# mryab/learning-at-home

Hardware: NVIDIA H100
Metric: DMoE training samples/sec (whole job, device-timed, max over ranks) (higher is better)
Workload: dtype bf16

## Files before the change

### learning-at-home_b200/csrc/small_m.cu

```cuda
#include "sm90.cuh"
#include <climits>

namespace lah {
namespace smallm {

constexpr int BM = 128;
constexpr int BK = 64;
constexpr int MMA_K = 16;
constexpr int BN_MAX = 128;
constexpr int NUM_THREADS = 288;

namespace sab {

constexpr int STAGES = 6;
constexpr int A_BYTES = BM * BK * 2;
constexpr int B_BYTES = BN_MAX * BK * 2;
constexpr int STAGE_BYTES = A_BYTES + B_BYTES;
constexpr int BAR_OFFSET = STAGES * STAGE_BYTES;
constexpr int QD = 4;
constexpr int MAX_G = 1023;
constexpr int CUM_OFFSET = BAR_OFFSET + (2 * STAGES + 2 * QD) * 8 + QD * 4 + 16;
constexpr int SMEM_TOTAL = CUM_OFFSET + (MAX_G + 1) * 4 + 1024;
static_assert(SMEM_TOTAL <= 232448, "shared memory budget");

struct Params {
    int G, M_out, K;
    const int* group_off;
    const int* group_rows;
    bf16* out;
    long long ldo;
    const float* bias;
    const bf16* residual;
    long long ldr;
    const int* wait_flags;
    int wait_count, wait_epoch;
    const int* epoch_base;
    int* status;
    int* tile_counter;
};

__device__ __forceinline__ int box_rows_of(int nn) { return nn <= 16 ? 16 : (nn <= 32 ? 32 : (nn <= 64 ? 64 : 128)); }

__device__ __forceinline__ int find_group(const int* cum, int G, int gc) {
    int lo = 0, hi = G - 1;
    while (lo < hi) {
        const int mid = (lo + hi + 1) >> 1;
        if (cum[mid] <= gc) lo = mid; else hi = mid - 1;
    }
    return lo;
}

template <int NB, bool A_MN>
__device__ __forceinline__ void sab_tile(const Params& p, uint8_t* smem, uint64_t* full_bar, uint64_t* empty_bar, int& stage,
                                         uint32_t& phase, int num_kb, int wg, int warp, int lane, int g, int ms, int row0,
// ... 141 lines not shown
                mbar_wait(&empty_bar[stage], phase ^ 1);
                uint8_t* sa = smem + stage * STAGE_BYTES;
                uint8_t* sb = sa + A_BYTES;
                const int k = kb * BK;
                mbar_arrive_expect_tx(&full_bar[stage], A_BYTES + box * 128);
                if (!A_MN) {
                    tma_load_3d(sa, &tmA, &full_bar[stage], k, ms * BM, g);
                } else {
#pragma unroll
                    for (int i = 0; i < BM / 64; ++i)
                        tma_load_3d(sa + i * (BK * 128), &tmA, &full_bar[stage], ms * BM + i * 64, k, g);
                }
                tma_load_2d(sb, tmB, &full_bar[stage], k, off + n0);
                if (++stage == STAGES) {
                    stage = 0;
                    phase ^= 1;
                }
            }
        }
        return;
    }

    const int wg = warp >> 2;
    int stage = 0, qi = 0;
    uint32_t phase = 0, qphase = 0;
    while (true) {
        mbar_wait(&q_full[qi], qphase);
        const int tile = q_tile[qi];
        __syncwarp();
        if (lane == 0) mbar_arrive(&q_empty[qi]);
        if (++qi == QD) {
            qi = 0;
            qphase ^= 1;
        }
        if (tile >= total) break;
        const int gc = tile / m_slices, ms = tile - gc * m_slices;
        const int g = find_group(cum, p.G, gc);
        const int n0 = (gc - cum[g]) * BN_MAX;
        const int nn = min(__ldg(p.group_rows + g) - n0, BN_MAX);
        const int row0 = __ldg(p.group_off + g) + n0;
        switch (box_rows_of(nn)) {
            case 16: sab_tile<16, A_MN>(p, smem, full_bar, empty_bar, stage, phase, num_kb, wg, warp, lane, g, ms, row0, nn); break;
            case 32: sab_tile<32, A_MN>(p, smem, full_bar, empty_bar, stage, phase, num_kb, wg, warp, lane, g, ms, row0, nn); break;
            case 64: sab_tile<64, A_MN>(p, smem, full_bar, empty_bar, stage, phase, num_kb, wg, warp, lane, g, ms, row0, nn); break;
            default: sab_tile<128, A_MN>(p, smem, full_bar, empty_bar, stage, phase, num_kb, wg, warp, lane, g, ms, row0, nn); break;
        }
    }
}

}

namespace wa {

constexpr int WBK = 32;
constexpr int OP_STAGES = 2;
constexpr int OP_STAGE_BYTES = 2 * (WBK * BM * 2);
constexpr int OP_BYTES = OP_STAGES * OP_STAGE_BYTES;
constexpr int CH_COLS = 32;
constexpr int CHUNKS = BN_MAX / CH_COLS;
constexpr int ARR_BYTES = BM * CH_COLS * 4;
constexpr int ST_STAGES = 3;
constexpr int ST_STAGE_BYTES = 4 * ARR_BYTES;
constexpr int ST_OFFSET = OP_BYTES;
constexpr int BAR_OFFSET = ST_OFFSET + ST_STAGES * ST_STAGE_BYTES;
constexpr int QD = 4;
constexpr int SMEM_TOTAL = BAR_OFFSET + (2 * OP_STAGES + 2 * ST_STAGES + 2 * QD) * 8 + QD * 4 + 16 + 1024;
static_assert(ST_STAGES <= CHUNKS, "the producer issues a tile's first ST_STAGES chunks before its remaining k-blocks");
static_assert(OP_STAGE_BYTES % 1024 == 0 && ARR_BYTES % 1024 == 0, "128-B swizzle atoms need 1 KB alignment");
static_assert(SMEM_TOTAL <= 232448, "shared memory budget");

struct Params {
    int G, N, K;
    const int* group_off;
    const int* group_rows;
    const int* skip;
    const int* step;
    float* p;
    float* m;
    float* v;
    float* vmax;
    bf16* p_bf16;
    float lr, beta1, beta2, eps;
    int amsgrad;
    float wd;
    int* tile_counter;
    const int* poison;
};

constexpr int WD_NONE = 0, WD_L2 = 1, WD_DECOUPLED = 2;

struct Tile {
    int g, mt, nt;
};

struct StateMaps {
    CUtensorMap a[4];
};

template <int WD>
__global__ void __launch_bounds__(NUM_THREADS, 1)
wgrad_adam_kernel(const Params p, const __grid_constant__ CUtensorMap tmDY, const __grid_constant__ CUtensorMap tmX,
                  const __grid_constant__ StateMaps tmS) {
    extern __shared__ uint8_t smem_raw[];
    uint8_t* smem = reinterpret_cast<uint8_t*>((reinterpret_cast<uintptr_t>(smem_raw) + 1023) & ~uintptr_t(1023));
    uint8_t* st_smem = smem + ST_OFFSET;
    uint64_t* op_full = reinterpret_cast<uint64_t*>(smem + BAR_OFFSET);
    uint64_t* op_empty = op_full + OP_STAGES;
    uint64_t* st_full = op_empty + OP_STAGES;
    uint64_t* st_empty = st_full + ST_STAGES;
    uint64_t* q_full = st_empty + ST_STAGES;
    uint64_t* q_empty = q_full + QD;
    volatile int* q_tile = reinterpret_cast<volatile int*>(q_empty + QD);

    const int warp = threadIdx.x >> 5;
    const int lane = threadIdx.x & 31;
    if (p.poison && (*p.poison & 1)) return;
    const int n_arr = p.amsgrad ? 4 : 3;

    if (warp == 8 && lane == 0) {
        tma_prefetch_desc(&tmDY);
        tma_prefetch_desc(&tmX);
        for (int a = 0; a < n_arr; ++a) tma_prefetch_desc(&tmS.a[a]);
        for (int i = 0; i < OP_STAGES; ++i) {
            mbar_init(&op_full[i], 1);
            mbar_init(&op_empty[i], 8);
        }
        for (int i = 0; i < ST_STAGES; ++i) {
            mbar_init(&st_full[i], 1);
            mbar_init(&st_empty[i], 1);
        }
        for (int i = 0; i < QD; ++i) {
            mbar_init(&q_full[i], 1);
            mbar_init(&q_empty[i], 8);
        }
        fence_mbar_init();
    }
    __syncthreads();

    const int n_tiles = p.K / BN_MAX;
    const int tiles_per_group = (p.N / BM) * n_tiles;
    const int total = p.G * tiles_per_group;
    auto decode = [&](int tile) {
        Tile t;
        t.g = tile / tiles_per_group;
        const int r = tile - t.g * tiles_per_group;
        t.mt = r / n_tiles;
        t.nt = r - t.mt * n_tiles;
        return t;
    };

    if (warp == 8) {
        if (lane != 0) return;
        uint32_t phase = 0, qphase = 0, sphase = 0;
        int qi = 0, stage = 0, sstage = 0;
        while (true) {
            int tile;
            while (true) {
                tile = atomicAdd(p.tile_counter, 1);
                if (tile >= total) break;
                const int g = tile / tiles_per_group;
                if (__ldg(p.group_rows + g) > 0 && !(p.skip && __ldg(p.skip + 2 * g) >= 0)) break;
                atomicMax(p.tile_counter, (g + 1) * tiles_per_group);
            }
            mbar_wait(&q_empty[qi], qphase ^ 1);
            q_tile[qi] = tile;
            mbar_arrive(&q_full[qi]);
            if (++qi == QD) {
                qi = 0;
                qphase ^= 1;
            }
            if (tile >= total) break;
            const Tile t = decode(tile);
            const int off = __ldg(p.group_off + t.g), rows = __ldg(p.group_rows + t.g);
            const int srow = t.g * p.N + t.mt * BM;
            auto load_chunk = [&](int c) {
                mbar_wait(&st_empty[sstage], sphase ^ 1);
                mbar_arrive_expect_tx(&st_full[sstage], n_arr * ARR_BYTES);
                uint8_t* ss = st_smem + sstage * ST_STAGE_BYTES;
                for (int a = 0; a < n_arr; ++a)
                    tma_load_2d(ss + a * ARR_BYTES, &tmS.a[a], &st_full[sstage], t.nt * BN_MAX + c * CH_COLS, srow);
                if (++sstage == ST_STAGES) {
                    sstage = 0;
                    sphase ^= 1;
                }
            };
            for (int t0 = 0; t0 < rows; t0 += WBK) {
                mbar_wait(&op_empty[stage], phase ^ 1);
                mbar_arrive_expect_tx(&op_full[stage], OP_STAGE_BYTES);
                uint8_t* sa = smem + stage * OP_STAGE_BYTES;
                uint8_t* sb = sa + WBK * BM * 2;
#pragma unroll
                for (int i = 0; i < BM / 64; ++i)
                    tma_load_2d(sa + i * (WBK * 128), &tmDY, &op_full[stage], t.mt * BM + i * 64, off + t0);
#pragma unroll
                for (int i = 0; i < BN_MAX / 64; ++i)
                    tma_load_2d(sb + i * (WBK * 128), &tmX, &op_full[stage], t.nt * BN_MAX + i * 64, off + t0);
                if (++stage == OP_STAGES) {
                    stage = 0;
                    phase ^= 1;
                }
                if (t0 == 0)
                    for (int c = 0; c < ST_STAGES; ++c) load_chunk(c);
            }
            for (int c = ST_STAGES; c < CHUNKS; ++c) load_chunk(c);
        }
        return;
    }

    const int wg = warp >> 2;
    int qi = 0, stage = 0, sstage = 0;
    uint32_t phase = 0, qphase = 0, sphase = 0;
    float acc[BN_MAX / 2];
    const int lrow = wg * 64 + (warp & 3) * 16 + (lane >> 2);
    const int sw = lrow & 7;
    while (true) {
        mbar_wait(&q_full[qi], qphase);
        const int tile = q_tile[qi];
        __syncwarp();
        if (lane == 0) mbar_arrive(&q_empty[qi]);
        if (++qi == QD) {
            qi = 0;
            qphase ^= 1;
        }
        if (tile >= total) break;
        const Tile t = decode(tile);
        const int rows = __ldg(p.group_rows + t.g);
        int prev_stage = -1;
        for (int t0 = 0; t0 < rows; t0 += WBK) {
            mbar_wait(&op_full[stage], phase);
            const uint32_t sa = smem_u32(smem + stage * OP_STAGE_BYTES) + wg * (WBK * 128);
            const uint32_t sb = smem_u32(smem + stage * OP_STAGE_BYTES + WBK * BM * 2);
            const int ksteps = min(WBK / MMA_K, (rows - t0 + MMA_K - 1) / MMA_K);
            wgmma_fence();
            for (int k = 0; k < ksteps; ++k) {
                const uint64_t da = make_smem_desc_sw128(sa + k * (MMA_K * 128), WBK * 128, 1024);
                const uint64_t db = make_smem_desc_sw128(sb + k * (MMA_K * 128), WBK * 128, 1024);
                wgmma_bf16_n128<1, 1>(acc, da, db, (t0 > 0 || k > 0) ? 1u : 0u);
            }
            wgmma_commit();
            wgmma_wait<1>();
            if (prev_stage >= 0) {
                __syncwarp();
                if (lane == 0) mbar_arrive(&op_empty[prev_stage]);
            }
            prev_stage = stage;
            if (++stage == OP_STAGES) {
                stage = 0;
                phase ^= 1;
            }
        }
        wgmma_wait<0>();
        wgmma_fence_regs(acc);
        __syncwarp();
        if (lane == 0 && prev_stage >= 0) mbar_arrive(&op_empty[prev_stage]);

        const float st = static_cast<float>(__ldg(p.step + t.g));
        const float step_size = p.lr / (1.f - powf(p.beta1, st));
        const float inv_sqrt_bc2 = rsqrtf(1.f - powf(p.beta2, st));
        const int srow = t.g * p.N + t.mt * BM;
        const long long row_base = static_cast<long long>(srow) + lrow;
        const int col_base = t.nt * BN_MAX + 2 * (lane & 3);
#pragma unroll
        for (int c = 0; c < CHUNKS; ++c) {
            mbar_wait(&st_full[sstage], sphase);
            uint8_t* ss = st_smem + sstage * ST_STAGE_BYTES;
#pragma unroll
            for (int jj = 0; jj < CH_COLS / 8; ++jj)
#pragma unroll
                for (int h = 0; h < 2; ++h) {
                    const int so = (lrow + 8 * h) * 128 + (((2 * jj + ((lane & 3) >> 1)) ^ sw) << 4) + 8 * (lane & 1);
                    float2* sp = reinterpret_cast<float2*>(ss + so);
                    float2* sm = reinterpret_cast<float2*>(ss + ARR_BYTES + so);
                    float2* sv = reinterpret_cast<float2*>(ss + 2 * ARR_BYTES + so);
                    float2* svm = reinterpret_cast<float2*>(ss + 3 * ARR_BYTES + so);
                    float2 pw = *sp, m = *sm, v = *sv;
                    float2 vm = p.amsgrad ? *svm : make_float2(0.f, 0.f);
                    float* pp = &pw.x; float* mp = &m.x; float* vp = &v.x; float* vmp = &vm.x;
#pragma unroll
                    for (int e = 0; e < 2; ++e) {
                        float grad = acc[4 * jj + 2 * h + e];
                        if constexpr (WD == WD_L2) grad += p.wd * pp[e];
                        if constexpr (WD == WD_DECOUPLED) pp[e] = __fmul_rn(pp[e], p.wd);
                        mp[e] = mp[e] + (1.f - p.beta1) * (grad - mp[e]);
                        vp[e] = vp[e] * p.beta2 + (1.f - p.beta2) * grad * grad;
                        float denom;
                        if (p.amsgrad) {
                            vmp[e] = fmaxf(vmp[e], vp[e]);
                            denom = sqrtf(vmp[e]) * inv_sqrt_bc2 + p.eps;
                        } else {
                            denom = sqrtf(vp[e]) * inv_sqrt_bc2 + p.eps;
                        }
                        pp[e] -= step_size * (mp[e] / denom);
                    }
                    *sp = pw;
                    *sm = m;
                    *sv = v;
                    if (p.amsgrad) *svm = vm;
                    const long long o = (row_base + 8 * h) * p.K + col_base + CH_COLS * c + 8 * jj;
                    *reinterpret_cast<uint32_t*>(p.p_bf16 + o) = pack_bf16x2(pw.x, pw.y);
                }
            fence_proxy_async_smem();
            named_bar_sync(1, 256);
            if (threadIdx.x == 0) {
                for (int a = 0; a < n_arr; ++a)
                    tma_store_2d(&tmS.a[a], ss + a * ARR_BYTES, t.nt * BN_MAX + c * CH_COLS, srow);
                tma_store_commit();
                tma_store_wait_read<0>();
                mbar_arrive(&st_empty[sstage]);
            }
            if (++sstage == ST_STAGES) {
                sstage = 0;
                sphase ^= 1;
            }
#pragma unroll
            for (int i = 0; i < BN_MAX / 2 - 16; ++i) acc[i] = acc[i + 16];
        }
    }
    if (threadIdx.x == 0) tma_store_wait<0>();
}

}
}
}

using namespace lah;
using namespace lah::smallm;

extern "C" const int* lah_get_epoch_base();

static int* tile_counter() {
    static int* ctr = nullptr;
    if (!ctr) {
        if (cudaMalloc(&ctr, 256) != cudaSuccess) return nullptr;
        cudaMemset(ctr, 0, 256);
    }
    return ctr;
}
static const int* g_poison = nullptr;

extern "C" {

int lah_set_poison_word(const int* status) {
    g_poison = status;
    return 0;
}
const int* lah_get_poison_word() { return g_poison; }

int lah_swapab_linear(const void* x, long long ldx, int x_rows, const void* W, int G, int M_out, int K, int a_mn,
                      void* out, long long ldo, const int* group_off, const int* group_rows, const float* bias,
                      const void* residual, long long ldr, const int* wait_flags, int wait_count, int wait_epoch,
                      const int* epoch_base, int* status, int max_ctas, cudaStream_t st) {
    if ((K % BK) || (M_out % BM) || (ldx % 8) || G > sab::MAX_G) return -2;
    CUtensorMap tmA, tmB[4];
    if (!a_mn) {
        uint64_t dims[3] = {(uint64_t)K, (uint64_t)M_out, (uint64_t)G};
        uint64_t str[2] = {(uint64_t)K * 2, (uint64_t)M_out * K * 2};
        uint32_t box[3] = {BK, BM, 1};
        int r = make_tmap(&tmA, CU_TENSOR_MAP_DATA_TYPE_BFLOAT16, 3, W, dims, str, box);
        if (r) return r;
    } else {
        uint64_t dims[3] = {(uint64_t)M_out, (uint64_t)K, (uint64_t)G};
        uint64_t str[2] = {(uint64_t)M_out * 2, (uint64_t)M_out * K * 2};
        uint32_t box[3] = {64, BK, 1};
        int r = make_tmap(&tmA, CU_TENSOR_MAP_DATA_TYPE_BFLOAT16, 3, W, dims, str, box);
        if (r) return r;
    }
    const uint32_t boxes[4] = {16, 32, 64, 128};
    for (int i = 0; i < 4; ++i) {
        uint64_t dims[2] = {(uint64_t)K, (uint64_t)x_rows};
        uint64_t str[1] = {(uint64_t)ldx * 2};
        uint32_t box[2] = {BK, boxes[i]};
        int r = make_tmap(&tmB[i], CU_TENSOR_MAP_DATA_TYPE_BFLOAT16, 2, x, dims, str, box);
        if (r) return r;
    }
    sab::Params p;
    p.G = G; p.M_out = M_out; p.K = K; p.group_off = group_off; p.group_rows = group_rows; p.out = (bf16*)out; p.ldo = ldo;
    p.bias = bias; p.residual = (const bf16*)residual; p.ldr = ldr; p.wait_flags = wait_flags; p.wait_count = wait_count;
    p.wait_epoch = wait_epoch; p.epoch_base = epoch_base ? epoch_base : lah_get_epoch_base(); p.status = status;
    p.tile_counter = tile_counter();
    if (!p.tile_counter) return -3;
    const long long total = 1ll * (M_out / BM) * (G + x_rows / BN_MAX);
    if (total <= 0 || G <= 0) return 0;
    if (cudaMemsetAsync(p.tile_counter, 0, sizeof(int), st) != cudaSuccess) return -4;
    const int ctas = persistent_grid(total, max_ctas);
    if (!a_mn) {
        if (int e = set_max_dynamic_smem<sab::swapab_kernel<false>>(sab::SMEM_TOTAL)) return e;
        sab::swapab_kernel<false><<<ctas, NUM_THREADS, sab::SMEM_TOTAL, st>>>(p, tmA, tmB[0], tmB[1], tmB[2], tmB[3]);
    } else {
        if (int e = set_max_dynamic_smem<sab::swapab_kernel<true>>(sab::SMEM_TOTAL)) return e;
        sab::swapab_kernel<true><<<ctas, NUM_THREADS, sab::SMEM_TOTAL, st>>>(p, tmA, tmB[0], tmB[1], tmB[2], tmB[3]);
    }
    return -(int)cudaGetLastError();
}

int lah_wgrad_adam_wd(const void* dy, long long lddy, const void* x, long long ldx, int total_rows, int G, int N, int K,
                      const int* group_off, const int* group_rows, const int* skip, const int* step, float* p, float* m,
                      float* v, float* vmax, void* p_bf16, float lr, float beta1, float beta2, float eps, int amsgrad,
                      float weight_decay, float decay, int max_ctas, cudaStream_t st) {
    if ((N % BM) || (K % BN_MAX) || (lddy % 8) || (ldx % 8) || 1ll * G * N > INT_MAX) return -2;
    if (decay != 1.f && weight_decay != 0.f) return -2;
    if (amsgrad && !vmax) return -2;
    CUtensorMap tmDY, tmX;
    wa::StateMaps tmS;
    {
        float* arrs[4] = {p, m, v, amsgrad ? vmax : p};
        uint64_t dims[2] = {(uint64_t)K, (uint64_t)G * N};
        uint64_t str[1] = {(uint64_t)K * 4};
        uint32_t box[2] = {wa::CH_COLS, BM};
        for (int a = 0; a < 4; ++a) {
            int r = make_tmap(&tmS.a[a], CU_TENSOR_MAP_DATA_TYPE_FLOAT32, 2, arrs[a], dims, str, box);
            if (r) return r;
        }
    }
    {
        uint64_t dims[2] = {(uint64_t)N, (uint64_t)total_rows};
        uint64_t str[1] = {(uint64_t)lddy * 2};
        uint32_t box[2] = {64, wa::WBK};
        int r = make_tmap(&tmDY, CU_TENSOR_MAP_DATA_TYPE_BFLOAT16, 2, dy, dims, str, box);
        if (r) return r;
    }
    {
        uint64_t dims[2] = {(uint64_t)K, (uint64_t)total_rows};
        uint64_t str[1] = {(uint64_t)ldx * 2};
        uint32_t box[2] = {64, wa::WBK};
        int r = make_tmap(&tmX, CU_TENSOR_MAP_DATA_TYPE_BFLOAT16, 2, x, dims, str, box);
        if (r) return r;
    }
    wa::Params a;
    a.G = G; a.N = N; a.K = K; a.group_off = group_off; a.group_rows = group_rows; a.skip = skip; a.step = step;
    a.p = p; a.m = m; a.v = v; a.vmax = vmax; a.p_bf16 = (bf16*)p_bf16; a.lr = lr; a.beta1 = beta1; a.beta2 = beta2; a.eps = eps; a.amsgrad = amsgrad;
    a.wd = decay != 1.f ? decay : weight_decay;
    a.tile_counter = tile_counter() ? tile_counter() + 16 : nullptr;
    a.poison = g_poison;
    if (!a.tile_counter) return -3;
    const long long total = 1ll * G * (N / BM) * (K / BN_MAX);
    if (total <= 0) return 0;
    if (cudaMemsetAsync(a.tile_counter, 0, sizeof(int), st) != cudaSuccess) return -4;
    const int ctas = persistent_grid(total, max_ctas);
    if (decay != 1.f) {
        if (int e = set_max_dynamic_smem<wa::wgrad_adam_kernel<wa::WD_DECOUPLED>>(wa::SMEM_TOTAL)) return e;
        wa::wgrad_adam_kernel<wa::WD_DECOUPLED><<<ctas, NUM_THREADS, wa::SMEM_TOTAL, st>>>(a, tmDY, tmX, tmS);
    } else if (weight_decay != 0.f) {
        if (int e = set_max_dynamic_smem<wa::wgrad_adam_kernel<wa::WD_L2>>(wa::SMEM_TOTAL)) return e;
        wa::wgrad_adam_kernel<wa::WD_L2><<<ctas, NUM_THREADS, wa::SMEM_TOTAL, st>>>(a, tmDY, tmX, tmS);
    } else {
        if (int e = set_max_dynamic_smem<wa::wgrad_adam_kernel<wa::WD_NONE>>(wa::SMEM_TOTAL)) return e;
        wa::wgrad_adam_kernel<wa::WD_NONE><<<ctas, NUM_THREADS, wa::SMEM_TOTAL, st>>>(a, tmDY, tmX, tmS);
    }
    return -(int)cudaGetLastError();
}

int lah_wgrad_adam(const void* dy, long long lddy, const void* x, long long ldx, int total_rows, int G, int N, int K,
                   const int* group_off, const int* group_rows, const int* skip, const int* step, float* p, float* m,
                   float* v, float* vmax, void* p_bf16, float lr, float beta1, float beta2, float eps, int amsgrad,
                   int max_ctas, cudaStream_t st) {
    return lah_wgrad_adam_wd(dy, lddy, x, ldx, total_rows, G, N, K, group_off, group_rows, skip, step, p, m, v, vmax, p_bf16,
                             lr, beta1, beta2, eps, amsgrad, 0.f, 1.f, max_ctas, st);
}

}
```

### learning-at-home_b200/parallel/engine.py

```python
import math
from dataclasses import dataclass, field
from typing import Dict, List, Optional, Sequence, Tuple

import torch
import torch.nn as nn
import torch.nn.functional as F

from ..ops import fp8, gemm, kernels as K, native

SEG_NAMES = ("w1", "b1", "g1", "be1", "w2", "b2", "g2", "be2", "w3", "b3")
REF_KEYS = {"w1": "layers.0.weight", "b1": "layers.0.bias", "g1": "layers.1.weight", "be1": "layers.1.bias",
            "w2": "layers.3.weight", "b2": "layers.3.bias", "g2": "layers.4.weight", "be2": "layers.4.bias",
            "w3": "layers.6.weight", "b3": "layers.6.bias"}
SMALL_SEG_MASK = sum(1 << i for i, n in enumerate(SEG_NAMES) if not n.startswith("w"))


@dataclass
class DMoEConfig:
    hidden: int = 512
    grid_size: Tuple[int, ...] = (8, 8)
    k: int = 4
    num_layers: int = 4
    in_features: int = 784
    num_classes: int = 10
    tokens_per_rank: int = 1024
    capacity_factor: float = 2.0
    failure_rate: float = 0.0
    lr: float = 1e-3
    betas: Tuple[float, float] = (0.9, 0.999)
    eps: float = 1e-8
    amsgrad: bool = True
    weight_decay: float = 0.0
    decoupled_weight_decay: bool = False
    seed: int = 1337
    uid_prefix: str = "expert"
    gate_mode: str = "product_key"
    shadow_experts: int = 8
    shadow_tol: float = 1.1
    shadow_min_rows: int = 1024
    expert_dtype: str = "bf16"
    expert_path: str = "auto"
    optimizer_ctas: int = -1
    update_every_inputs: int = 0
    update_every_steps: int = 0
    trainer_staleness: int = 0
    trainer_microbatches: int = 1
    peer_timeout_ms: int = 0

    def resolved_path(self, world: int = 1) -> str:
        if self.accumulate:
            return "big"
        if self.expert_path != "auto":
            return self.expert_path
        rows_per_expert = self.tokens_per_rank * world * self.k / max(1, self.num_experts)
        experts_per_rank = -(-self.num_experts // max(1, world))
        return "small" if (rows_per_expert < 512 and self.expert_dtype == "bf16" and self.inner % 128 == 0
                           and self.hidden % 128 == 0
                           and experts_per_rank <= 1023) else "big"

    @property
    def accumulate(self) -> bool:
        return self.update_every_inputs > 1 or self.update_every_steps > 1

    def update_thresholds(self) -> Tuple[int, int]:
        never = 2 ** 31 - 1
        return (self.update_every_inputs if self.update_every_inputs > 0 else never,
                self.update_every_steps if self.update_every_steps > 0 else never)
# ... 26 lines not shown

class EngineContext:

    def __init__(self, cfg: DMoEConfig, group=None, device=None, heap_bytes: Optional[int] = None):
        from .symmetric import SymmetricHeap
        import torch.distributed as dist
        self.cfg = cfg
        self.device = device or torch.device("cuda", torch.cuda.current_device())
        distributed = dist.is_available() and dist.is_initialized()
        self.world = dist.get_world_size(group) if distributed else 1
        self.rank = dist.get_rank(group) if distributed else 0
        assert cfg.num_experts % self.world == 0, "experts must divide evenly over ranks"
        self.E = cfg.num_experts
        self.E_loc = self.E // self.world
        pairs = cfg.tokens_per_rank * cfg.k
        cap = pairs if self.world == 1 else int(math.ceil(pairs * cfg.capacity_factor))
        self.small = cfg.resolved_path(self.world) == "small"
        if self.small:
            self.align = self.tile_rows = 16
            self.S = 0
        else:
            self.align = 256 if cfg.hidden % 256 == 0 and cfg.inner % 256 == 0 else 128
            self.tile_rows = 128
            self.S = min(int(cfg.shadow_experts), 2 * K.MAX_WORLD) if self.world > 1 else 0
        self.G_tot = self.E_loc + self.S
        self.max_rows = ((cap + self.align - 1) // self.align + self.G_tot) * self.align
        self.max_rows = (self.max_rows + 127) // 128 * 128
        self.max_tiles = self.max_rows // self.tile_rows
        H = cfg.hidden
        sym_rows_bytes = self.max_rows * H * 2
        need = (3 * cfg.num_layers + 2) * (sym_rows_bytes + 4096) + K.MAX_WORLD * self.E * 4 + (32 << 20)
        if self.S:
            rec = sum(int(math.prod(shape)) for shape in cfg.seg_shapes().values())
            need += cfg.num_layers * (self.G_tot * rec * 10 + (1 << 20))
        self.heap = SymmetricHeap(heap_bytes or need, group=group, device=self.device)
        self.flags, self.flags_off = self.heap.alloc((K.NUM_SLOTS, K.MAX_WORLD), torch.int32)
        self.cnt_all, self.cnt_all_off = self.heap.alloc((K.MAX_WORLD, self.E), torch.int32)
        i32 = dict(dtype=torch.int32, device=self.device)
        self.counts = torch.zeros(self.E, **i32)
        self.done_counter = torch.zeros(1, **i32)
        self._status_buf = torch.zeros(4, **i32)
        self.status = self._status_buf[:1]
        self.wait_ns = self._status_buf[2:4].view(torch.int64)
        K.set_wait_counter(self.wait_ns)
        self.step_ctr = torch.zeros(4, **i32)
        K.set_step_counters(self.step_ctr)
        K.set_spin_timeout_ms(cfg.peer_timeout_ms)
        self.step_ctr[1] = int(cfg.peer_timeout_ms)
        self.dead_mask = 0
        import os as _os
        octas = int(_os.environ.get("LAH_OPTIMIZER_CTAS", cfg.optimizer_ctas))
        sms = torch.cuda.get_device_properties(self.device).multi_processor_count
        if octas < 0:
            octas = sms * (17 if self.world == 1 else 18) // 28
        self.opt_ctas = octas if (self.small and 0 < octas < sms - 8) else 0
        self.chain_ctas = sms - self.opt_ctas if self.opt_ctas else 0
        self.opt_stream = torch.cuda.Stream(self.device) if self.opt_ctas else None
        self._opt_pending = False
        self.defer_join = False
        K.set_poison_word(self.status)
        assert 2 * cfg.num_layers + 4 < self.EPOCH_STRIDE
        self.alive = torch.ones(self.E, dtype=torch.uint8, device=self.device)
        self.hb, self.hb_off = self.heap.alloc((self.E,), torch.int64)
        self.hb.zero_()
        self._hb_stream = None
        self.epoch = 0
        self.token_counter = 0
        from .profiler import StageTimer
        self.timer = StageTimer(enabled=False)
        self.gyd, self.gyd_off = self.heap.alloc((self.max_rows, H), torch.bfloat16)
        self.dxd, self.dxd_off = self.heap.alloc((self.max_rows, H), torch.bfloat16)
        bf = dict(dtype=torch.bfloat16, device=self.device)
        self.da = torch.empty(self.max_rows, cfg.inner, **bf)
        self.dh = torch.empty(self.max_rows, cfg.inner, **bf)
        self.heap.barrier()

    EPOCH_STRIDE = 64

    def close(self):
        K.set_wait_counter(None)
        K.set_step_counters(None)
        K.set_poison_word(None)
        self.heap.close()

    def heartbeat(self, experts=None, now: Optional[float] = None):
        import time
        first, count = experts if experts is not None else (self.rank * self.E_loc, self.E_loc)
        now_ms = int((time.time() if now is None else now) * 1000)
        if self._hb_stream is None:
            self._hb_stream = torch.cuda.Stream(self.device)
        with torch.cuda.stream(self._hb_stream):
            K.heartbeat(self.hb_off, first, count, now_ms)

    def refresh_alive(self, heartbeat_expiration: float = 120.0, now: Optional[float] = None):
        import time
        now_ms = int((time.time() if now is None else now) * 1000)
        if self._hb_stream is None:
            self._hb_stream = torch.cuda.Stream(self.device)
        with torch.cuda.stream(self._hb_stream):
            K.alive_from_heartbeats(self.hb, self.alive, now_ms, int(heartbeat_expiration * 1000))
            self._apply_dead_mask()

    def step_failed(self) -> bool:
        return bool(int(self.status.item()) & K.STATUS_TIMEOUT)

    def clear_failure(self):
        self._status_buf[0] = 0
# ... 580 lines not shown
```

### learning-at-home_b200/build_native.py

```python
import hashlib
import os
import shutil
import subprocess
import sys
from pathlib import Path

ROOT = Path(__file__).resolve().parent
CSRC = ROOT / "csrc"
OUT = ROOT / "_C"

NVCC_FLAGS = [
    "-gencode", "arch=compute_90a,code=sm_90a", "-lineinfo", "-O3", "-std=c++17",
    "--use_fast_math", "-Xcompiler", "-fPIC", "-Xcompiler", "-fvisibility=default",
]
GXX_FLAGS = ["-O3", "-std=c++17", "-fPIC", "-shared", "-pthread", "-Wall"]


def _nvcc() -> str:
    for cand in (os.environ.get("NVCC"), shutil.which("nvcc"), "/usr/local/cuda/bin/nvcc"):
        if cand and os.path.exists(cand):
            return cand
    raise RuntimeError("nvcc not found")


# ... 17 lines not shown
    if res.returncode != 0:
        sys.stderr.write(res.stdout + res.stderr)
        raise RuntimeError(f"native build failed: {' '.join(map(str, cmd[:3]))} ...")
    if verbose and (res.stdout or res.stderr):
        print(res.stdout + res.stderr)


def build_cuda(force=False, verbose=False, ptxas_verbose=False) -> Path:
    OUT.mkdir(exist_ok=True)
    target = OUT / "liblah_cuda.so"
    cus = sorted(CSRC.glob("*.cu"))
    hdrs = sorted(CSRC.glob("*.cuh")) + sorted(CSRC.glob("*.h"))
    digest = _digest(cus + hdrs, " ".join(NVCC_FLAGS))
    if not force and not _needs_build(target, digest):
        return target
    objs = []
    procs = []
    objdir = OUT / "obj"
    objdir.mkdir(exist_ok=True)
    for cu in cus:
        obj = objdir / (cu.stem + ".o")
        cmd = [_nvcc(), *NVCC_FLAGS, *( ["-Xptxas", "-v"] if ptxas_verbose else []), "-I", CSRC, "-c", cu, "-o", obj]
        if verbose:
            print("+", " ".join(map(str, cmd)), flush=True)
        procs.append((cu, subprocess.Popen(list(map(str, cmd)), stdout=subprocess.PIPE, stderr=subprocess.STDOUT, text=True)))
        objs.append(obj)
    for cu, proc in procs:
        out, _ = proc.communicate()
        if proc.returncode != 0:
            sys.stderr.write(out)
            raise RuntimeError(f"nvcc failed on {cu.name}")
        if (verbose or ptxas_verbose) and out:
            print(out)
    _run([_nvcc(), "-shared", "-o", target, *objs], verbose)
    target.with_suffix(".so.stamp").write_text(digest)
    return target


def build_host(force=False, verbose=False) -> Path:
    OUT.mkdir(exist_ok=True)
    target = OUT / "liblah_host.so"
    cpps = sorted(CSRC.glob("*.cpp"))
    hdrs = sorted(CSRC.glob("*.hpp"))
    if not cpps:
        return target
    digest = _digest(cpps + hdrs, " ".join(GXX_FLAGS))
    if not force and not _needs_build(target, digest):
        return target
    _run(["g++", *GXX_FLAGS, "-I", CSRC, "-o", target, *cpps], verbose)
    target.with_suffix(".so.stamp").write_text(digest)
    return target


def build_all(force=False, verbose=False):
    return build_cuda(force, verbose), build_host(force, verbose)


if __name__ == "__main__":
    force = "--force" in sys.argv
    c, h = build_cuda(force, verbose=True, ptxas_verbose="--ptxas" in sys.argv), build_host(force, verbose=True)
    print("built:", c, h)
```

Before: 12670.

## Split fused wgrad-Adam state pipeline into per-warp row chunks with vectorized bf16 stores

The optimizer-state TMA pipeline in the fused wgrad+Adam kernel is re-chunked from column strips across all 256 consumer threads into 16-row chunks, one per consumer warp, with six stages. Each warp now waits, updates and stores its own chunk independently, so the per-chunk 256-thread barrier and the single-thread store bottleneck go away. The bf16 mirror writes become 16-byte stores after warp shuffles. The tile counter now resets itself at kernel end instead of through a separate memset, and the default optimizer CTA share for single-rank runs rises. The cost is more TMA boxes per chunk and a more intricate phase-tracking scheme.

```diff
diff --git a/learning-at-home_b200/csrc/small_m.cu b/learning-at-home_b200/csrc/small_m.cu
--- a/learning-at-home_b200/csrc/small_m.cu
+++ b/learning-at-home_b200/csrc/small_m.cu
@@ -251,17 +251,20 @@
 constexpr int OP_STAGES = 2;
 constexpr int OP_STAGE_BYTES = 2 * (WBK * BM * 2);
 constexpr int OP_BYTES = OP_STAGES * OP_STAGE_BYTES;
-constexpr int CH_COLS = 32;
-constexpr int CHUNKS = BN_MAX / CH_COLS;
-constexpr int ARR_BYTES = BM * CH_COLS * 4;
-constexpr int ST_STAGES = 3;
+constexpr int CH_ROWS = 16;
+constexpr int CHUNKS = BM / CH_ROWS;
+constexpr int BOX_COLS = 32;
+constexpr int BOX_BYTES = CH_ROWS * BOX_COLS * 4;
+constexpr int ARR_BYTES = (BN_MAX / BOX_COLS) * BOX_BYTES;
+constexpr int ST_STAGES = 6;
 constexpr int ST_STAGE_BYTES = 4 * ARR_BYTES;
 constexpr int ST_OFFSET = OP_BYTES;
 constexpr int BAR_OFFSET = ST_OFFSET + ST_STAGES * ST_STAGE_BYTES;
 constexpr int QD = 4;
 constexpr int SMEM_TOTAL = BAR_OFFSET + (2 * OP_STAGES + 2 * ST_STAGES + 2 * QD) * 8 + QD * 4 + 16 + 1024;
+static_assert(CHUNKS == 8, "one chunk per consumer warp");
 static_assert(ST_STAGES <= CHUNKS, "the producer issues a tile's first ST_STAGES chunks before its remaining k-blocks");
-static_assert(OP_STAGE_BYTES % 1024 == 0 && ARR_BYTES % 1024 == 0, "128-B swizzle atoms need 1 KB alignment");
+static_assert(OP_STAGE_BYTES % 1024 == 0 && BOX_BYTES % 1024 == 0, "128-B swizzle atoms need 1 KB alignment");
 static_assert(SMEM_TOTAL <= 232448, "shared memory budget");
 
 struct Params {
@@ -346,8 +349,8 @@
 
     if (warp == 8) {
         if (lane != 0) return;
-        uint32_t phase = 0, qphase = 0, sphase = 0;
-        int qi = 0, stage = 0, sstage = 0;
+        uint32_t phase = 0, qphase = 0;
+        int qi = 0, stage = 0, nload = 0;
         while (true) {
             int tile;
             while (true) {
@@ -369,15 +372,16 @@
             const int off = __ldg(p.group_off + t.g), rows = __ldg(p.group_rows + t.g);
             const int srow = t.g * p.N + t.mt * BM;
             auto load_chunk = [&](int c) {
-                mbar_wait(&st_empty[sstage], sphase ^ 1);
-                mbar_arrive_expect_tx(&st_full[sstage], n_arr * ARR_BYTES);
-                uint8_t* ss = st_smem + sstage * ST_STAGE_BYTES;
+                const int slot = nload % ST_STAGES;
+                mbar_wait(&st_empty[slot], ((nload / ST_STAGES) & 1) ^ 1);
+                mbar_arrive_expect_tx(&st_full[slot], n_arr * ARR_BYTES);
+                uint8_t* ss = st_smem + slot * ST_STAGE_BYTES;
                 for (int a = 0; a < n_arr; ++a)
-                    tma_load_2d(ss + a * ARR_BYTES, &tmS.a[a], &st_full[sstage], t.nt * BN_MAX + c * CH_COLS, srow);
-                if (++sstage == ST_STAGES) {
-                    sstage = 0;
-                    sphase ^= 1;
-                }
+#pragma unroll
+                    for (int b = 0; b < BN_MAX / BOX_COLS; ++b)
+                        tma_load_2d(ss + a * ARR_BYTES + b * BOX_BYTES, &tmS.a[a], &st_full[slot],
+                                    t.nt * BN_MAX + b * BOX_COLS, srow + c * CH_ROWS);
+                ++nload;
             };
             for (int t0 = 0; t0 < rows; t0 += WBK) {
                 mbar_wait(&op_empty[stage], phase ^ 1);
@@ -399,15 +403,19 @@
             }
             for (int c = ST_STAGES; c < CHUNKS; ++c) load_chunk(c);
         }
+        __threadfence();
+        if (atomicAdd(p.tile_counter + 1, 1) == static_cast<int>(gridDim.x) - 1) {
+            p.tile_counter[0] = 0;
+            p.tile_counter[1] = 0;
+        }
         return;
     }
 
     const int wg = warp >> 2;
-    int qi = 0, stage = 0, sstage = 0;
-    uint32_t phase = 0, qphase = 0, sphase = 0;
+    int qi = 0, stage = 0, nchunk = 0;
+    uint32_t phase = 0, qphase = 0;
     float acc[BN_MAX / 2];
-    const int lrow = wg * 64 + (warp & 3) * 16 + (lane >> 2);
-    const int sw = lrow & 7;
+    const int r = lane >> 2;
     while (true) {
         mbar_wait(&q_full[qi], qphase);
         const int tile = q_tile[qi];
@@ -452,18 +460,24 @@
         const float st = static_cast<float>(__ldg(p.step + t.g));
         const float step_size = p.lr / (1.f - powf(p.beta1, st));
         const float inv_sqrt_bc2 = rsqrtf(1.f - powf(p.beta2, st));
-        const int srow = t.g * p.N + t.mt * BM;
-        const long long row_base = static_cast<long long>(srow) + lrow;
-        const int col_base = t.nt * BN_MAX + 2 * (lane & 3);
-#pragma unroll
-        for (int c = 0; c < CHUNKS; ++c) {
-            mbar_wait(&st_full[sstage], sphase);
-            uint8_t* ss = st_smem + sstage * ST_STAGE_BYTES;
-#pragma unroll
-            for (int jj = 0; jj < CH_COLS / 8; ++jj)
+        const int crow = t.g * p.N + t.mt * BM + warp * CH_ROWS;
+        named_bar_sync(1, 256);
+        const int n = nchunk + warp;
+        const int slot = n % ST_STAGES;
+        const uint32_t use = n / ST_STAGES;
+        mbar_wait(&st_empty[slot], (use & 1) ^ 1);
+        mbar_wait(&st_full[slot], use & 1);
+        nchunk += CHUNKS;
+        uint8_t* ss = st_smem + slot * ST_STAGE_BYTES;
+#pragma unroll
+        for (int b = 0; b < BN_MAX / BOX_COLS; ++b) {
+            uint32_t mirror[2][4];
+#pragma unroll
+            for (int jj = 0; jj < BOX_COLS / 8; ++jj)
 #pragma unroll
                 for (int h = 0; h < 2; ++h) {
-                    const int so = (lrow + 8 * h) * 128 + (((2 * jj + ((lane & 3) >> 1)) ^ sw) << 4) + 8 * (lane & 1);
+                    const int so = b * BOX_BYTES + (r + 8 * h) * 128 + (((2 * jj + ((lane & 3) >> 1)) ^ r) << 4) +
+                                   8 * (lane & 1);
                     float2* sp = reinterpret_cast<float2*>(ss + so);
                     float2* sm = reinterpret_cast<float2*>(ss + ARR_BYTES + so);
                     float2* sv = reinterpret_cast<float2*>(ss + 2 * ARR_BYTES + so);
@@ -473,7 +487,7 @@
                     float* pp = &pw.x; float* mp = &m.x; float* vp = &v.x; float* vmp = &vm.x;
 #pragma unroll
                     for (int e = 0; e < 2; ++e) {
-                        float grad = acc[4 * jj + 2 * h + e];
+                        float grad = acc[16 * b + 4 * jj + 2 * h + e];
                         if constexpr (WD == WD_L2) grad += p.wd * pp[e];
                         if constexpr (WD == WD_DECOUPLED) pp[e] = __fmul_rn(pp[e], p.wd);
                         mp[e] = mp[e] + (1.f - p.beta1) * (grad - mp[e]);
@@ -491,27 +505,39 @@
                     *sm = m;
                     *sv = v;
                     if (p.amsgrad) *svm = vm;
-                    const long long o = (row_base + 8 * h) * p.K + col_base + CH_COLS * c + 8 * jj;
-                    *reinterpret_cast<uint32_t*>(p.p_bf16 + o) = pack_bf16x2(pw.x, pw.y);
+                    mirror[h][jj] = pack_bf16x2(pw.x, pw.y);
                 }
-            fence_proxy_async_smem();
-            named_bar_sync(1, 256);
-            if (threadIdx.x == 0) {
-                for (int a = 0; a < n_arr; ++a)
-                    tma_store_2d(&tmS.a[a], ss + a * ARR_BYTES, t.nt * BN_MAX + c * CH_COLS, srow);
-                tma_store_commit();
-                tma_store_wait_read<0>();
-                mbar_arrive(&st_empty[sstage]);
-            }
-            if (++sstage == ST_STAGES) {
-                sstage = 0;
-                sphase ^= 1;
-            }
-#pragma unroll
-            for (int i = 0; i < BN_MAX / 2 - 16; ++i) acc[i] = acc[i + 16];
-        }
-    }
-    if (threadIdx.x == 0) tma_store_wait<0>();
+            const int q = lane & 3;
+#pragma unroll
+            for (int h = 0; h < 2; ++h) {
+                uint32_t* w = mirror[h];
+#pragma unroll
+                for (int k = 0; k < 2; ++k) {
+                    const uint32_t got = __shfl_xor_sync(0xffffffffu, (q & 2) ? w[k] : w[k + 2], 2);
+                    if (q & 2) w[k] = got; else w[k + 2] = got;
+                }
+#pragma unroll
+                for (int k = 0; k < 2; ++k) {
+                    const uint32_t got = __shfl_xor_sync(0xffffffffu, (q & 1) ? w[2 * k] : w[2 * k + 1], 1);
+                    if (q & 1) w[2 * k] = got; else w[2 * k + 1] = got;
+                }
+                const long long o = static_cast<long long>(crow + r + 8 * h) * p.K + t.nt * BN_MAX + b * BOX_COLS + 8 * q;
+                *reinterpret_cast<uint4*>(p.p_bf16 + o) = make_uint4(w[0], w[1], w[2], w[3]);
+            }
+        }
+        fence_proxy_async_smem();
+        __syncwarp();
+        if (lane == 0) {
+            for (int a = 0; a < n_arr; ++a)
+#pragma unroll
+                for (int b = 0; b < BN_MAX / BOX_COLS; ++b)
+                    tma_store_2d(&tmS.a[a], ss + a * ARR_BYTES + b * BOX_BYTES, t.nt * BN_MAX + b * BOX_COLS, crow);
+            tma_store_commit();
+            tma_store_wait_read<0>();
+            mbar_arrive(&st_empty[slot]);
+        }
+    }
+    if (lane == 0) tma_store_wait<0>();
 }
 
 }
@@ -601,7 +627,7 @@
         float* arrs[4] = {p, m, v, amsgrad ? vmax : p};
         uint64_t dims[2] = {(uint64_t)K, (uint64_t)G * N};
         uint64_t str[1] = {(uint64_t)K * 4};
-        uint32_t box[2] = {wa::CH_COLS, BM};
+        uint32_t box[2] = {wa::BOX_COLS, wa::CH_ROWS};
         for (int a = 0; a < 4; ++a) {
             int r = make_tmap(&tmS.a[a], CU_TENSOR_MAP_DATA_TYPE_FLOAT32, 2, arrs[a], dims, str, box);
             if (r) return r;
@@ -630,7 +656,6 @@
     if (!a.tile_counter) return -3;
     const long long total = 1ll * G * (N / BM) * (K / BN_MAX);
     if (total <= 0) return 0;
-    if (cudaMemsetAsync(a.tile_counter, 0, sizeof(int), st) != cudaSuccess) return -4;
     const int ctas = persistent_grid(total, max_ctas);
     if (decay != 1.f) {
         if (int e = set_max_dynamic_smem<wa::wgrad_adam_kernel<wa::WD_DECOUPLED>>(wa::SMEM_TOTAL)) return e;
diff --git a/learning-at-home_b200/parallel/engine.py b/learning-at-home_b200/parallel/engine.py
--- a/learning-at-home_b200/parallel/engine.py
+++ b/learning-at-home_b200/parallel/engine.py
@@ -13,6 +13,10 @@
             "w2": "layers.3.weight", "b2": "layers.3.bias", "g2": "layers.4.weight", "be2": "layers.4.bias",
             "w3": "layers.6.weight", "b3": "layers.6.bias"}
 SMALL_SEG_MASK = sum(1 << i for i, n in enumerate(SEG_NAMES) if not n.startswith("w"))
+
+
+def default_optimizer_ctas(sms: int, world: int) -> int:
+    return sms * (21 if world == 1 else 18) // 28
 
 
 @dataclass
@@ -145,7 +149,7 @@
         octas = int(_os.environ.get("LAH_OPTIMIZER_CTAS", cfg.optimizer_ctas))
         sms = torch.cuda.get_device_properties(self.device).multi_processor_count
         if octas < 0:
-            octas = sms * (17 if self.world == 1 else 18) // 28
+            octas = default_optimizer_ctas(sms, self.world)
         self.opt_ctas = octas if (self.small and 0 < octas < sms - 8) else 0
         self.chain_ctas = sms - self.opt_ctas if self.opt_ctas else 0
         self.opt_stream = torch.cuda.Stream(self.device) if self.opt_ctas else None
```

After: 13060 (median of 6 runs). 3.1% higher.

## Stage bf16 weight mirror in swizzled smem and store via TMA; shrink wgrad k-block

Applied to the files above, without the earlier changes.

The fused wgrad+Adam epilogue no longer writes the bf16 parameter mirror with scattered per-thread global stores. It packs values into registers, stages them in a 64B-swizzled shared buffer, and issues a TMA tensor store alongside the fp32 state stores. The operand pipeline also changes from two stages of 32-row k-blocks to three stages of 16-row k-blocks. A standalone probe library is built to benchmark state-streaming variants. The extra named barrier per chunk adds sync cost, and the smaller k-block means more barrier round trips.

```diff
diff --git a/learning-at-home_b200/build_native.py b/learning-at-home_b200/build_native.py
--- a/learning-at-home_b200/build_native.py
+++ b/learning-at-home_b200/build_native.py
@@ -93,8 +93,23 @@
     return target
 
 
+def build_probe(force=False, verbose=False) -> Path:
+    OUT.mkdir(exist_ok=True)
+    target = OUT / "liblah_probe.so"
+    srcs = sorted((CSRC / "probe").glob("*.cu")) + [CSRC / "small_m.cu", CSRC / "sm90.cuh"]
+    flags = [*NVCC_FLAGS, "-DLAH_WA_RELEASE_AFTER_STORE_READ=0"]
+    digest = _digest(srcs, " ".join(flags))
+    if not force and not _needs_build(target, digest):
+        return target
+    _run([_nvcc(), *flags, "-shared", "-I", CSRC, "-o", target, *sorted((CSRC / "probe").glob("*.cu"))], verbose)
+    target.with_suffix(".so.stamp").write_text(digest)
+    return target
+
+
 def build_all(force=False, verbose=False):
-    return build_cuda(force, verbose), build_host(force, verbose)
+    cuda_so, host_so = build_cuda(force, verbose), build_host(force, verbose)
+    build_probe(force, verbose)
+    return cuda_so, host_so
 
 
 if __name__ == "__main__":
diff --git a/learning-at-home_b200/csrc/probe/optimizer_stream_probe.cu b/learning-at-home_b200/csrc/probe/optimizer_stream_probe.cu
--- /dev/null
+++ b/learning-at-home_b200/csrc/probe/optimizer_stream_probe.cu
@@ -0,0 +1,255 @@
+#include "small_m.cu"
+
+namespace lah {
+namespace probe {
+
+using smallm::BM;
+using smallm::NUM_THREADS;
+constexpr int CH_COLS = 32;
+constexpr int CHUNKS = 128 / CH_COLS;
+constexpr int ARR_BYTES = BM * CH_COLS * 4;
+constexpr int MIR_BYTES = BM * CH_COLS * 2;
+constexpr int ST_STAGES = 3;
+constexpr int STAGE_BYTES = 4 * ARR_BYTES + MIR_BYTES;
+constexpr int BAR_OFFSET = ST_STAGES * STAGE_BYTES;
+constexpr int SMEM_TOTAL = BAR_OFFSET + 2 * ST_STAGES * 8 + ST_STAGES * 8 + 1024;
+static_assert(SMEM_TOTAL <= 232448, "shared memory budget");
+
+struct Params {
+    int G, N, K;
+    float* arr[4];
+    bf16* p_bf16;
+    int* tile_counter;
+};
+
+struct Maps {
+    CUtensorMap a[4];
+    CUtensorMap mirror;
+    CUtensorMap b64[4], b32[4];
+};
+
+__device__ __forceinline__ void bulk_load(void* dst, const void* src, uint32_t bytes, uint64_t* bar) {
+    asm volatile("cp.async.bulk.shared::cluster.global.mbarrier::complete_tx::bytes [%0], [%1], %2, [%3];"
+                 ::"r"(smem_u32(dst)), "l"(src), "r"(bytes), "r"(smem_u32(bar)) : "memory");
+}
+__device__ __forceinline__ void bulk_store(void* dst, const void* src, uint32_t bytes) {
+    asm volatile("cp.async.bulk.global.shared::cta.bulk_group [%0], [%1], %2;" ::"l"(dst), "r"(smem_u32(src)), "r"(bytes)
+                 : "memory");
+}
+
+template <int LAYOUT, int MIRROR, int RELEASE>
+__global__ void __launch_bounds__(NUM_THREADS, 1) state_stream_kernel(const Params p, const __grid_constant__ Maps tm) {
+    extern __shared__ uint8_t smem_raw[];
+    uint8_t* smem = reinterpret_cast<uint8_t*>((reinterpret_cast<uintptr_t>(smem_raw) + 1023) & ~uintptr_t(1023));
+    uint64_t* full = reinterpret_cast<uint64_t*>(smem + BAR_OFFSET);
+    uint64_t* empty = full + ST_STAGES;
+    int2* coord = reinterpret_cast<int2*>(empty + ST_STAGES);
+    const int warp = threadIdx.x >> 5, lane = threadIdx.x & 31;
+    if (warp == 8 && lane == 0) {
+        for (int i = 0; i < ST_STAGES; ++i) {
+            mbar_init(&full[i], 1);
+            mbar_init(&empty[i], 1);
+        }
+        fence_mbar_init();
+    }
+    __syncthreads();
+    const int n_tiles = p.K / 128;
+    const int tiles_per_group = (p.N / BM) * n_tiles;
+    const int total = p.G * tiles_per_group;
+
+    if (warp == 8) {
+        if (lane != 0) return;
+        int s = 0;
+        uint32_t ph = 0;
+        auto next_slot = [&]() {
+            if (++s == ST_STAGES) {
+                s = 0;
+                ph ^= 1;
+            }
+        };
+        while (true) {
+            const int tile = atomicAdd(p.tile_counter, 1);
+            if (tile >= total) break;
+            const int g = tile / tiles_per_group, r = tile - g * tiles_per_group;
+            const int mt = r / n_tiles, nt = r - mt * n_tiles;
+            for (int c = 0; c < CHUNKS; ++c) {
+                mbar_wait(&empty[s], ph ^ 1);
+                uint8_t* ss = smem + s * STAGE_BYTES;
+                mbar_arrive_expect_tx(&full[s], 4 * ARR_BYTES);
+                if (LAYOUT >= 2) {
+                    constexpr int RB = LAYOUT == 2 ? 64 : 32;
+                    coord[s] = LAYOUT == 2 ? make_int2(nt * 128 + (c >> 1) * 64, g * p.N + mt * BM + (c & 1) * 64)
+                                           : make_int2(nt * 128, g * p.N + mt * BM + c * 32);
+                    for (int a = 0; a < 4; ++a)
+                        for (int b = 0; b < BM / RB; ++b)
+                            tma_load_2d(ss + a * ARR_BYTES + b * (RB * 128), LAYOUT == 2 ? &tm.b64[a] : &tm.b32[a], &full[s],
+                                        coord[s].x + 32 * b, coord[s].y);
+                } else if (LAYOUT == 0) {
+                    coord[s] = make_int2(nt * 128 + c * CH_COLS, g * p.N + mt * BM);
+                    for (int a = 0; a < 4; ++a) tma_load_2d(ss + a * ARR_BYTES, &tm.a[a], &full[s], coord[s].x, coord[s].y);
+                } else {
+                    const long long e0 = (static_cast<long long>(tile) * CHUNKS + c) * (BM * CH_COLS);
+                    coord[s] = make_int2(static_cast<int>(e0 & 0x3fffffff), static_cast<int>(e0 >> 30));
+                    for (int a = 0; a < 4; ++a) bulk_load(ss + a * ARR_BYTES, p.arr[a] + e0, ARR_BYTES, &full[s]);
+                }
+                next_slot();
+            }
+        }
+        mbar_wait(&empty[s], ph ^ 1);
+        coord[s] = make_int2(-1, -1);
+        mbar_arrive(&full[s]);
+        return;
+    }
+
+    const int wg = warp >> 2;
+    const int lrow = wg * 64 + (warp & 3) * 16 + (lane >> 2);
+    const int sw = lrow & 7;
+    int s = 0, prev = -1;
+    uint32_t ph = 0;
+    while (true) {
+        mbar_wait(&full[s], ph);
+        const int2 xy = coord[s];
+        if (xy.x < 0) break;
+        uint8_t* ss = smem + s * STAGE_BYTES;
+        if (MIRROR) {
+#pragma unroll
+            for (int jj = 0; jj < CH_COLS / 8; ++jj)
+#pragma unroll
+                for (int h = 0; h < 2; ++h) {
+                    const int so = (lrow + 8 * h) * 128 + (((2 * jj + ((lane & 3) >> 1)) ^ sw) << 4) + 8 * (lane & 1);
+                    const float2 pw = *reinterpret_cast<const float2*>(ss + so);
+                    const int row = lrow + 8 * h;
+                    if (MIRROR == 1) {
+                        const long long o = static_cast<long long>(xy.y + row) * p.K + xy.x + 8 * jj + 2 * (lane & 3);
+                        *reinterpret_cast<uint32_t*>(p.p_bf16 + o) = pack_bf16x2(pw.x, pw.y);
+                    } else {
+                        const int mo = row * 64 + ((jj ^ ((row >> 1) & 3)) << 4) + 4 * (lane & 3);
+                        *reinterpret_cast<uint32_t*>(ss + 4 * ARR_BYTES + mo) = pack_bf16x2(pw.x, pw.y);
+                    }
+                }
+        }
+        fence_proxy_async_smem();
+        named_bar_sync(1, 256);
+        if (threadIdx.x == 0) {
+            if (LAYOUT >= 2) {
+                constexpr int RB = LAYOUT == 2 ? 64 : 32;
+                for (int a = 0; a < 4; ++a)
+                    for (int b = 0; b < BM / RB; ++b)
+                        tma_store_2d(LAYOUT == 2 ? &tm.b64[a] : &tm.b32[a], ss + a * ARR_BYTES + b * (RB * 128), xy.x + 32 * b,
+                                     xy.y);
+            } else if (LAYOUT == 0) {
+                for (int a = 0; a < 4; ++a) tma_store_2d(&tm.a[a], ss + a * ARR_BYTES, xy.x, xy.y);
+                if (MIRROR == 2) tma_store_2d(&tm.mirror, ss + 4 * ARR_BYTES, xy.x, xy.y);
+            } else {
+                const long long e0 = (static_cast<long long>(xy.y) << 30) | xy.x;
+                for (int a = 0; a < 4; ++a) bulk_store(p.arr[a] + e0, ss + a * ARR_BYTES, ARR_BYTES);
+            }
+            tma_store_commit();
+            if (RELEASE == 0) {
+                tma_store_wait_read<0>();
+                mbar_arrive(&empty[s]);
+            } else if (RELEASE == 1) {
+                mbar_arrive(&empty[s]);
+            } else {
+                tma_store_wait_read<1>();
+                if (prev >= 0) mbar_arrive(&empty[prev]);
+            }
+        }
+        prev = s;
+        if (++s == ST_STAGES) {
+            s = 0;
+            ph ^= 1;
+        }
+    }
+    if (threadIdx.x == 0) tma_store_wait<0>();
+}
+
+__global__ void copy_kernel(const int4* __restrict__ src, int4* __restrict__ dst, long long n) {
+    const long long stride = static_cast<long long>(gridDim.x) * blockDim.x;
+    long long i = static_cast<long long>(blockIdx.x) * blockDim.x + threadIdx.x;
+    for (; i + 3 * stride < n; i += 4 * stride) {
+        const int4 a = src[i], b = src[i + stride], c = src[i + 2 * stride], d = src[i + 3 * stride];
+        dst[i] = a;
+        dst[i + stride] = b;
+        dst[i + 2 * stride] = c;
+        dst[i + 3 * stride] = d;
+    }
+    for (; i < n; i += stride) dst[i] = src[i];
+}
+
+template <int LAYOUT, int MIRROR, int RELEASE>
+int launch(const Params& p, const Maps& tm, int ctas, cudaStream_t st) {
+    if (int e = set_max_dynamic_smem<state_stream_kernel<LAYOUT, MIRROR, RELEASE>>(SMEM_TOTAL)) return e;
+    state_stream_kernel<LAYOUT, MIRROR, RELEASE><<<ctas, NUM_THREADS, SMEM_TOTAL, st>>>(p, tm);
+    return -static_cast<int>(cudaGetLastError());
+}
+
+}
+}
+
+extern "C" {
+
+const int* lah_get_epoch_base() { return nullptr; }
+
+int probe_state_stream(int variant, float* p0, float* m0, float* v0, float* vm0, void* p_bf16, int G, int N, int K,
+                       int max_ctas, cudaStream_t st) {
+    using namespace lah::probe;
+    if ((N % BM) || (K % 128) || G <= 0) return -2;
+    Params p;
+    p.G = G; p.N = N; p.K = K; p.arr[0] = p0; p.arr[1] = m0; p.arr[2] = v0; p.arr[3] = vm0; p.p_bf16 = (lah::bf16*)p_bf16;
+    static int* ctr = nullptr;
+    if (!ctr && cudaMalloc(&ctr, 256) != cudaSuccess) return -3;
+    p.tile_counter = ctr;
+    Maps tm;
+    for (int a = 0; a < 4; ++a) {
+        uint64_t dims[2] = {(uint64_t)K, (uint64_t)G * N};
+        uint64_t str[1] = {(uint64_t)K * 4};
+        uint32_t box[2] = {CH_COLS, BM};
+        if (int r = lah::make_tmap(&tm.a[a], CU_TENSOR_MAP_DATA_TYPE_FLOAT32, 2, p.arr[a], dims, str, box)) return r;
+        uint32_t box64[2] = {CH_COLS, 64}, box32[2] = {CH_COLS, 32};
+        if (int r = lah::make_tmap(&tm.b64[a], CU_TENSOR_MAP_DATA_TYPE_FLOAT32, 2, p.arr[a], dims, str, box64)) return r;
+        if (int r = lah::make_tmap(&tm.b32[a], CU_TENSOR_MAP_DATA_TYPE_FLOAT32, 2, p.arr[a], dims, str, box32)) return r;
+    }
+    {
+        uint64_t dims[2] = {(uint64_t)K, (uint64_t)G * N};
+        uint64_t str[1] = {(uint64_t)K * 2};
+        uint32_t box[2] = {CH_COLS, BM};
+        if (int r = lah::make_tmap(&tm.mirror, CU_TENSOR_MAP_DATA_TYPE_BFLOAT16, 2, p_bf16, dims, str, box,
+                                   CU_TENSOR_MAP_SWIZZLE_64B))
+            return r;
+    }
+    if (cudaMemsetAsync(ctr, 0, sizeof(int), st) != cudaSuccess) return -4;
+    const int ctas = lah::persistent_grid(1ll * G * (N / BM) * (K / 128), max_ctas);
+    switch (variant) {
+        case 0: return launch<0, 0, 0>(p, tm, ctas, st);
+        case 1: return launch<0, 0, 1>(p, tm, ctas, st);
+        case 2: return launch<0, 0, 2>(p, tm, ctas, st);
+        case 10: return launch<0, 1, 0>(p, tm, ctas, st);
+        case 20: return launch<0, 2, 0>(p, tm, ctas, st);
+        case 22: return launch<0, 2, 2>(p, tm, ctas, st);
+        case 200: return launch<2, 0, 0>(p, tm, ctas, st);
+        case 300: return launch<3, 0, 0>(p, tm, ctas, st);
+        case 100: return launch<1, 0, 0>(p, tm, ctas, st);
+        case 101: return launch<1, 0, 1>(p, tm, ctas, st);
+        default: return -2;
+    }
+}
+
+int probe_prepare_fused() {
+    using namespace lah::smallm::wa;
+    const cudaError_t e[3] = {
+        cudaFuncSetAttribute(wgrad_adam_kernel<WD_NONE>, cudaFuncAttributeMaxDynamicSharedMemorySize, SMEM_TOTAL),
+        cudaFuncSetAttribute(wgrad_adam_kernel<WD_L2>, cudaFuncAttributeMaxDynamicSharedMemorySize, SMEM_TOTAL),
+        cudaFuncSetAttribute(wgrad_adam_kernel<WD_DECOUPLED>, cudaFuncAttributeMaxDynamicSharedMemorySize, SMEM_TOTAL)};
+    for (cudaError_t x : e)
+        if (x != cudaSuccess) return -static_cast<int>(x);
+    return 0;
+}
+
+int probe_copy(const void* src, void* dst, long long bytes, int ctas, cudaStream_t st) {
+    if (bytes % 16) return -2;
+    lah::probe::copy_kernel<<<ctas, 1024, 0, st>>>((const int4*)src, (int4*)dst, bytes / 16);
+    return -static_cast<int>(cudaGetLastError());
+}
+
+}
diff --git a/learning-at-home_b200/csrc/small_m.cu b/learning-at-home_b200/csrc/small_m.cu
--- a/learning-at-home_b200/csrc/small_m.cu
+++ b/learning-at-home_b200/csrc/small_m.cu
@@ -1,5 +1,9 @@
 #include "sm90.cuh"
 #include <climits>
+
+#ifndef LAH_WA_RELEASE_AFTER_STORE_READ
+#define LAH_WA_RELEASE_AFTER_STORE_READ 1
+#endif
 
 namespace lah {
 namespace smallm {
@@ -247,8 +251,8 @@
 
 namespace wa {
 
-constexpr int WBK = 32;
-constexpr int OP_STAGES = 2;
+constexpr int WBK = 16;
+constexpr int OP_STAGES = 3;
 constexpr int OP_STAGE_BYTES = 2 * (WBK * BM * 2);
 constexpr int OP_BYTES = OP_STAGES * OP_STAGE_BYTES;
 constexpr int CH_COLS = 32;
@@ -257,11 +261,14 @@
 constexpr int ST_STAGES = 3;
 constexpr int ST_STAGE_BYTES = 4 * ARR_BYTES;
 constexpr int ST_OFFSET = OP_BYTES;
-constexpr int BAR_OFFSET = ST_OFFSET + ST_STAGES * ST_STAGE_BYTES;
+constexpr int MIR_OFFSET = ST_OFFSET + ST_STAGES * ST_STAGE_BYTES;
+constexpr int MIR_BYTES = BM * CH_COLS * 2;
+constexpr int BAR_OFFSET = MIR_OFFSET + MIR_BYTES;
 constexpr int QD = 4;
 constexpr int SMEM_TOTAL = BAR_OFFSET + (2 * OP_STAGES + 2 * ST_STAGES + 2 * QD) * 8 + QD * 4 + 16 + 1024;
 static_assert(ST_STAGES <= CHUNKS, "the producer issues a tile's first ST_STAGES chunks before its remaining k-blocks");
-static_assert(OP_STAGE_BYTES % 1024 == 0 && ARR_BYTES % 1024 == 0, "128-B swizzle atoms need 1 KB alignment");
+static_assert(OP_STAGE_BYTES % 1024 == 0 && ARR_BYTES % 1024 == 0 && MIR_OFFSET % 1024 == 0,
+              "swizzle atoms need 1 KB alignment");
 static_assert(SMEM_TOTAL <= 232448, "shared memory budget");
 
 struct Params {
@@ -274,7 +281,6 @@
     float* m;
     float* v;
     float* vmax;
-    bf16* p_bf16;
     float lr, beta1, beta2, eps;
     int amsgrad;
     float wd;
@@ -290,6 +296,7 @@
 
 struct StateMaps {
     CUtensorMap a[4];
+    CUtensorMap mirror;
 };
 
 template <int WD>
@@ -316,6 +323,7 @@
         tma_prefetch_desc(&tmDY);
         tma_prefetch_desc(&tmX);
         for (int a = 0; a < n_arr; ++a) tma_prefetch_desc(&tmS.a[a]);
+        tma_prefetch_desc(&tmS.mirror);
         for (int i = 0; i < OP_STAGES; ++i) {
             mbar_init(&op_full[i], 1);
             mbar_init(&op_empty[i], 8);
@@ -453,12 +461,11 @@
         const float step_size = p.lr / (1.f - powf(p.beta1, st));
         const float inv_sqrt_bc2 = rsqrtf(1.f - powf(p.beta2, st));
         const int srow = t.g * p.N + t.mt * BM;
-        const long long row_base = static_cast<long long>(srow) + lrow;
-        const int col_base = t.nt * BN_MAX + 2 * (lane & 3);
 #pragma unroll
         for (int c = 0; c < CHUNKS; ++c) {
             mbar_wait(&st_full[sstage], sphase);
             uint8_t* ss = st_smem + sstage * ST_STAGE_BYTES;
+            uint32_t mir[CH_COLS / 8][2];
 #pragma unroll
             for (int jj = 0; jj < CH_COLS / 8; ++jj)
 #pragma unroll
@@ -491,16 +498,25 @@
                     *sm = m;
                     *sv = v;
                     if (p.amsgrad) *svm = vm;
-                    const long long o = (row_base + 8 * h) * p.K + col_base + CH_COLS * c + 8 * jj;
-                    *reinterpret_cast<uint32_t*>(p.p_bf16 + o) = pack_bf16x2(pw.x, pw.y);
+                    mir[jj][h] = pack_bf16x2(pw.x, pw.y);
+                }
+            named_bar_sync(1, 256);
+#pragma unroll
+            for (int jj = 0; jj < CH_COLS / 8; ++jj)
+#pragma unroll
+                for (int h = 0; h < 2; ++h) {
+                    const int r = lrow + 8 * h;
+                    *reinterpret_cast<uint32_t*>(smem + MIR_OFFSET + r * 64 + ((jj ^ ((r >> 1) & 3)) << 4) + 4 * (lane & 3)) =
+                        mir[jj][h];
                 }
             fence_proxy_async_smem();
             named_bar_sync(1, 256);
             if (threadIdx.x == 0) {
                 for (int a = 0; a < n_arr; ++a)
                     tma_store_2d(&tmS.a[a], ss + a * ARR_BYTES, t.nt * BN_MAX + c * CH_COLS, srow);
+                tma_store_2d(&tmS.mirror, smem + MIR_OFFSET, t.nt * BN_MAX + c * CH_COLS, srow);
                 tma_store_commit();
-                tma_store_wait_read<0>();
+                if (LAH_WA_RELEASE_AFTER_STORE_READ) tma_store_wait_read<0>();
                 mbar_arrive(&st_empty[sstage]);
             }
             if (++sstage == ST_STAGES) {
@@ -606,6 +622,10 @@
             int r = make_tmap(&tmS.a[a], CU_TENSOR_MAP_DATA_TYPE_FLOAT32, 2, arrs[a], dims, str, box);
             if (r) return r;
         }
+        uint64_t str_bf16[1] = {(uint64_t)K * 2};
+        int r = make_tmap(&tmS.mirror, CU_TENSOR_MAP_DATA_TYPE_BFLOAT16, 2, p_bf16, dims, str_bf16, box,
+                          CU_TENSOR_MAP_SWIZZLE_64B);
+        if (r) return r;
     }
     {
         uint64_t dims[2] = {(uint64_t)N, (uint64_t)total_rows};
@@ -623,7 +643,7 @@
     }
     wa::Params a;
     a.G = G; a.N = N; a.K = K; a.group_off = group_off; a.group_rows = group_rows; a.skip = skip; a.step = step;
-    a.p = p; a.m = m; a.v = v; a.vmax = vmax; a.p_bf16 = (bf16*)p_bf16; a.lr = lr; a.beta1 = beta1; a.beta2 = beta2; a.eps = eps; a.amsgrad = amsgrad;
+    a.p = p; a.m = m; a.v = v; a.vmax = vmax; a.lr = lr; a.beta1 = beta1; a.beta2 = beta2; a.eps = eps; a.amsgrad = amsgrad;
     a.wd = decay != 1.f ? decay : weight_decay;
     a.tile_counter = tile_counter() ? tile_counter() + 16 : nullptr;
     a.poison = g_poison;
```

After: 12320 before, 12560 after (median of 6 runs). +1.9%, better.
